# jkulhanek/tetra-nerf

Hardware: AMD Instinct MI355X
Metric: ray_tet_intersections_per_s (higher is better)
Workload: dtype f32

## Files before the change

### tetra-nerf_amd/csrc/tn_api_tracer.hip

```cpp
#include <algorithm>
#include <cmath>
#include <cstring>
#include <memory>
#include <mutex>

#include "tn_api_common.h"
#include "tn_build.h"
#include "tn_devbuf.h"
#include "tn_isosurface_core.h"
#include "tn_kernels.h"

using tn::check_loaded;
using tn::check_pow2_M;
using tn::DeviceGuard;
using tn::guarded;

struct tn_tracer {
    int device = 0;
    std::mutex mu;

    struct Mesh {
        bool loaded = false;
        tn::DeviceMesh view;
        tn::HostMesh host;
// ... 15 lines not shown
        unsigned leaf_width = 16;
        int writer_table = 0;
        bool refit_tables = false;
        int use_walk = 1;
        size_t walk_min_rays = 12288;
        bool walk_min_auto = true;
        bool dense_tails = true;
        bool literal = true;
        size_t log_cap_bytes = 0;
        int spec_fill = 0;
        unsigned spec_k0 = 0;
        tn::FillRange spec{true, 0, true, tn::FillKind::Spans, 512};
        unsigned walk_lds_kb = 26;
        tn::FillRange tail{false, 0, false, tn::FillKind::RowPerBlock, 0};
        unsigned writer_blocks = 0;
        bool hull_flat = true;
        bool small_lds = true;
        unsigned lds_cap = 0;
        unsigned verify_stride = 256;
        bool verify_risk = true;
        unsigned risk_band = 2;
        bool verify_inject = false;
        unsigned literal_sort_passes = 8;
        int cert_ends = 2;
        bool bin_rays = false;
        bool timing = false;
    } opt;

    struct Scratch {
        tn::DevBuf<uint32_t> fallback_list;
        tn::DevBuf<uint32_t> walk_n;
        tn::DevBuf<uint4> hull_entry;
        tn::DevBuf<uint2> literal_list;
        tn::DevBuf<uint4> hit_log;
        tn::DevBuf<uint32_t> verify_list;
        tn::DevBuf<uint32_t> risk_list;
        tn::DevBuf<uint32_t> ray_keys, ray_iota, ray_keys_sorted, order, walk_n_item;
        tn::DevBuf<char> sort_temp;
        static constexpr int N_CTR = 2;
        tn::DevBuf<unsigned long long> stats;
        uint32_t *fallback_count() { return reinterpret_cast<uint32_t *>(stats.p + tn::N_STATS); }
        uint32_t *literal_count() { return fallback_count() + 1; }
        uint32_t *verify_count() { return fallback_count() + 2; }
        uint32_t *risk_count() { return fallback_count() + 3; }
        static constexpr size_t stats_bytes() { return (tn::N_STATS + N_CTR) * sizeof(unsigned long long); }
        size_t last_num_rays = 0;
        bool last_walk = false;
        bool last_binned = false;
        hipStream_t last_stream = nullptr;

        template <typename T>
        static void grow(tn::DevBuf<T> &b, size_t n) { if (b.n < n) b.alloc(n); }
        void reserve(size_t R, size_t log_entries, bool verify, bool risk, size_t sort_temp_bytes = 0) {
            grow(fallback_list, R);
            if (!log_entries) return;
            grow(walk_n, R); grow(literal_list, R); grow(hull_entry, R); grow(hit_log, log_entries);
            if (verify) grow(verify_list, R);
            if (risk) grow(risk_list, R);
            if (sort_temp_bytes) {
                grow(ray_keys, R); grow(ray_iota, R); grow(ray_keys_sorted, R); grow(order, R); grow(walk_n_item, R);
                grow(sort_temp, sort_temp_bytes);
            }
        }
    } scratch;

    struct Schedule {
        hipStream_t side = nullptr;
// ... 134 lines not shown
        w.risk_band = (float)o().risk_band;
        if (binned) { w.order = s().order.p; w.walk_n_item = s().walk_n_item.p; }
        w.cert_ends = o().cert_ends == 2 ? (m.T >= tn::WALK_TET_MIN_TETS ? 1u : 3u) : (uint32_t)o().cert_ends;
        return w;
    }
    tn::WriteParams write_params(size_t base, size_t n) const {
        const tn::Rows r = rows.at(base);
        tn::WriteParams q{};
        q.num_rays = n; q.M = r.M; q.dense_tails = dense_tails ? 1u : 0u;
        q.walk_n = s().walk_n.p + base;
        q.hit_log = s().hit_log.p;
        q.cold = mesh().cold; q.tets = mesh().tets;
        q.out_cells = r.cells; q.out_bary = r.bary; q.out_dist = r.dist; q.out_verts = r.verts;
        if (binned) { q.walk_n = s().walk_n_item.p; q.order = s().order.p; }
        return q;
    }

    void fill_tails(size_t base, size_t n, uint32_t k_hi) const {
        if (!dense_tails) return;
        tn::FillRange f = o().tail;
        f.k_split = k_hi;
        tn::launch_fill(rows.at(base), n, s().walk_n.p + base, f, stream);
    }
    void pair_literal(size_t base, size_t n, hipStream_t st) const {
        if (!o().literal) return;
        tn::launch_postprocess_log(trace_params(base, n), mesh().fidt, s().hit_log.p, s().literal_list.p, s().literal_count(), n, st,
                                   binned ? s().order.p : nullptr);
    }
    void trace_listed(const uint32_t *list, const uint32_t *count, size_t max_items, hipStream_t st) const {
        tn::TraceParams q = trace_params(0, max_items);
        q.ray_list = list; q.item_count = count;
        tn::launch_trace_general(q, st);
    }

    uint32_t spec_fill_first_slot() const {
        if (!o().spec_fill || !dense_tails) return 0;
        const uint32_t M = rows.M;
        uint32_t K0 = (((uint32_t)(3.6 * std::cbrt((double)std::max<uint32_t>(mesh().T, 1u))) + 31u) & ~31u) + 32u;
        const uint32_t quarter = (3u * M / 4u) & ~31u, half = (M / 2u) & ~31u;
        if (mesh().T >= tn::WALK_TET_MIN_TETS) K0 = K0 > quarter + 32u ? 0u : quarter;
        else K0 = K0 > quarter ? 0u : (K0 + 32u > half ? half : quarter);
        if (o().spec_k0) K0 = o().spec_k0 & ~31u;
        return K0 + 32u > M ? 0u : K0;
    }

    void run_overlapped() const {
        tn_tracer::Schedule &c = t->sched;
        const bool timing = o().timing;
        const hipStream_t s_pre = timing ? stream : c.pre, s_aux = timing ? stream : c.aux, s_side = timing ? stream : c.side;
        if (timing && !c.tev[0])
// ... 33 lines not shown
        }
        mark();
        TN_HIP(hipEventRecord(c.ev_aux, s_aux));
        tn::launch_write_segments(write_params(0, R), stream, o().writer_blocks);
        mark();
        TN_HIP(hipEventRecord(c.ev_seg, stream));
        TN_HIP(hipStreamWaitEvent(s_side, c.ev_seg, 0));
        pair_literal(0, R, s_side);
        mark();
        fill_tails(0, R, K0 ? K0 : rows.M);
        mark();
        TN_HIP(hipEventRecord(c.ev_join, s_side));
        TN_HIP(hipStreamWaitEvent(stream, c.ev_join, 0));
        TN_HIP(hipStreamWaitEvent(stream, c.ev_aux, 0));
        if (o().verify_stride) trace_listed(s().verify_list.p, s().verify_count(), 64, stream);
        mark();
        c.tev_valid = timing;
    }

    void run_chunked(size_t chunk) const {
        for (size_t base = 0; base < R; base += chunk) {
            const size_t n = std::min(R - base, chunk);
            TN_HIP(hipMemsetAsync(s().literal_count(), 0, sizeof(uint32_t), stream));
            TN_HIP(hipMemsetAsync(s().risk_count(), 0, sizeof(uint32_t), stream));
            const tn::WalkParams w = walk_params(base, n);
            tn::launch_trace_walk(w, stream, 0);
            if (o().verify_stride) {
                tn::launch_verify_counts(w.t, o().verify_stride, w.walk_n, w.fallback_list, w.fallback_count, base, stream, false,
                                         o().verify_inject);
                if (verify_risk())
                    tn::launch_verify_counts(w.t, o().verify_stride, w.walk_n, w.fallback_list, w.fallback_count, base, stream, false,
                                             false, s().risk_list.p, s().risk_count(), n);
            }
            tn::launch_write_segments(write_params(base, n), stream, o().writer_blocks);
            fill_tails(base, n, rows.M);
            pair_literal(base, n, stream);
        }
        trace_listed(s().fallback_list.p, s().fallback_count(), R, stream);
    }

    void run_small_batch() const {
        uint32_t C = 64;
        const double expect = 3.6 * std::cbrt((double)std::max<uint32_t>(mesh().T, 1u));
        while (C < expect && C < rows.M) C <<= 1;
        if (o().lds_cap) C = o().lds_cap;
        tn::TraceParams p = trace_params(0, R);
        if (o().small_lds && C < rows.M) {
// ... 600 lines not shown
            o.leaf_width = (unsigned)value;
        }
        else if (k == "walk") o.use_walk = value < 0 ? 0 : (value > 2 ? 2 : value);
        else if (k == "walk_min_rays") { o.walk_min_rays = value < 0 ? 0 : (size_t)value; o.walk_min_auto = false; }
        else if (k == "dense_tails") o.dense_tails = value != 0;
        else if (k == "literal") o.literal = value != 0;
        else if (k == "spec_fill") o.spec_fill = value != 0;
        else if (k == "spec_k0") o.spec_k0 = (unsigned)value;
        else if (k == "spec_blocks") set_grid(o.spec, value);
        else if (k == "hull_flat") o.hull_flat = value != 0;
        else if (k == "writer_blocks") o.writer_blocks = (unsigned)value;
        else if (k == "fill_blocks") set_grid(o.tail, value);
        else if (k == "walk_lds_kb") o.walk_lds_kb = (unsigned)value;
        else if (k == "small_lds") o.small_lds = value != 0;
        else if (k == "lds_cap") {
            if (value < 0 || (value & (value - 1)) != 0 || (value && value < 8)) throw tn::Error("lds_cap must be 0 or a power of two >= 8");
            o.lds_cap = (unsigned)value;
        }
        else if (k == "writer_table") o.writer_table = value;
        else if (k == "refit_tables") o.refit_tables = value != 0;
        else if (k == "cert_ends") { if (value < 0 || value > 3) throw tn::Error("cert_ends must be 0 .. 3"); o.cert_ends = value; }
        else if (k == "verify_inject") o.verify_inject = value != 0;
        else if (k == "literal_sort_passes") o.literal_sort_passes = value < 0 ? 0u : (unsigned)value;
        else if (k == "verify_stride") o.verify_stride = value < 0 ? 0u : (unsigned)value;
        else if (k == "verify_risk") o.verify_risk = value != 0;
        else if (k == "risk_band") o.risk_band = value < 1 ? 1u : (unsigned)value;
        else if (k == "log_cap_mb") o.log_cap_bytes = value <= 0 ? 0 : (size_t)value << 20;
        else throw tn::Error("unknown option " + (name ? k : std::string("(null)")));
    });
}

}
```

### tetra-nerf_amd/csrc/tn_kernels.h

```cpp
#pragma once
#include "tn_common.h"
#include "tn_ray_key.h"

namespace tn {

struct Rows {
    uint32_t *num;
    uint32_t *cells;
    float *bary;
    float *dist;
    uint32_t *verts;
    uint32_t M;
    Rows at(size_t base) const {
        return Rows{num ? num + base : nullptr, cells + base * M, bary + base * M * 6, dist + base * M * 2,
                    verts ? verts + base * M * 4 : nullptr, M};
    }
};

struct TraceParams {
    const float *origins;
    const float *dirs;
    const uint32_t *faces;
    const uint32_t *face_tets;
    WideBvh bvh;
// ... 32 lines not shown
    const float4 *hull_nodes;
    const float4 *hull_tris;
    uint32_t n_hull_nodes;
    const float4 *hull_flat;
    uint32_t n_hull_groups, n_hull_leaves;
    uint32_t n_hull;
    uint4 *hull_entry;
    uint32_t *fallback_list;
    uint32_t *fallback_count;
    uint2 *literal_list;
    uint32_t *literal_count;
    uint32_t *walk_n;
    uint4 *hit_log;
    size_t ray_base;
    uint32_t *risk_list;
    uint32_t *risk_count;
    float risk_band;
    uint32_t cert_ends;
    const uint32_t *order;
    uint32_t *walk_n_item;
};
void launch_trace_walk(const WalkParams &p, hipStream_t stream, size_t lds_reserve = 0);
void launch_postprocess_log(const TraceParams &p, const WalkFid *fidt, const uint4 *hit_log, const uint2 *literal_list,
                            const uint32_t *literal_count, size_t max_items, hipStream_t stream, const uint32_t *order = nullptr);

void launch_verify_counts(const TraceParams &p, uint32_t stride, uint32_t *walk_n, uint32_t *fallback_list, uint32_t *fallback_count,
                          size_t ray_base, hipStream_t stream, bool late = false, bool inject = false, const uint32_t *ray_list = nullptr,
                          const uint32_t *list_count = nullptr, size_t max_list = 0);

struct WriteParams {
    size_t num_rays;
    uint32_t M;
    uint32_t dense_tails;
    const uint32_t *walk_n;
    const uint4 *hit_log;
    const WalkCold *cold;
    const WalkTet *tets;
    uint32_t *out_cells;
    float *out_bary;
    float *out_dist;
    uint32_t *out_verts;
    const uint32_t *order;
};
void launch_write_segments(const WriteParams &q, hipStream_t stream, unsigned max_blocks = 0);
enum class FillKind {
    Spans,
    RowPerBlock,
// ... 189 lines not shown
```

### tetra-nerf_amd/csrc/tn_trace_general.hip

```cpp
#include "tn_device.h"
#include "tn_kernels.h"

namespace tn {

namespace {

struct WaveSmem {
    uint64_t *key;
    float *hu;
    float *hv;
    uint2 *hft;
    uint32_t *stack;
    uint8_t *mark;
    uint8_t *emitf;
};

__device__ __forceinline__ WaveSmem carve(char *smem, uint32_t M) {
    WaveSmem s;
    s.key = reinterpret_cast<uint64_t *>(smem);
    s.hft = reinterpret_cast<uint2 *>(s.key + M);
    s.hu = reinterpret_cast<float *>(s.hft + (M < 32 ? 32 : M));
    s.hv = s.hu + M;
    s.stack = reinterpret_cast<uint32_t *>(s.hv + M);
    s.mark = reinterpret_cast<uint8_t *>(s.stack + STACK_CAP);
    s.emitf = s.mark + M;
    return s;
}

__device__ __forceinline__ void wave_sync() { __syncthreads(); }

__device__ void insert_overflow(WaveSmem &s, uint32_t cap, uint64_t k, float u, float v, int lane) {
    uint64_t best = 0;
    uint32_t bidx = 0;
    for (uint32_t i = lane; i < cap; i += 64) {
        const uint64_t x = s.key[i];
        if (x >= best) { best = x; bidx = i; }
    }
#pragma unroll
    for (int off = 32; off > 0; off >>= 1) {
        const uint64_t ob = __shfl_xor(best, off);
        const uint32_t oi = __shfl_xor(bidx, off);
        if (ob > best || (ob == best && oi > bidx)) { best = ob; bidx = oi; }
    }
    if (k < best && lane == 0) { s.key[bidx] = k; s.hu[bidx] = u; s.hv[bidx] = v; }
    wave_sync();
}

__device__ void postprocess_and_write(const WaveSmem &s, uint32_t nh, uint32_t M, const uint32_t *__restrict__ faces,
                                      const uint32_t *__restrict__ face_tets, uint32_t *__restrict__ out_num,
                                      uint32_t *__restrict__ out_cells, float *__restrict__ out_bary,
                                      float *__restrict__ out_dist, uint32_t *__restrict__ out_verts,
                                      unsigned long long *stats, int lane, bool compact = false) {
    for (uint32_t base = 0; base < nh; base += 512) {
        uint2 ft[8];
#pragma unroll
        for (int q = 0; q < 8; ++q) {
            const uint32_t j = base + 64 * q + lane;
            if (j < nh) ft[q] = *reinterpret_cast<const uint2 *>(face_tets + 2 * (size_t)(uint32_t)s.key[j]);
        }
#pragma unroll
        for (int q = 0; q < 8; ++q) {
            const uint32_t j = base + 64 * q + lane;
            if (j < nh) { s.hft[j] = ft[q]; s.mark[j] = 0; }
        }
    }
    wave_sync();

    bool bad = false;
    for (uint32_t j = lane; j + 1 < nh; j += 64) {
        uint32_t c;
        const float t0 = __uint_as_float((uint32_t)(s.key[j] >> 32));
        const float t1 = __uint_as_float((uint32_t)(s.key[j + 1] >> 32));
        if (!common_tet(s.hft[j], s.hft[j + 1], c)) bad = true;
        if (j + 2 < nh) {
            const float t2 = __uint_as_float((uint32_t)(s.key[j + 2] >> 32));
            if (fabsf(t1 - t0) < TN_EPS && fabsf(t2 - t1) < TN_EPS) bad = true;
        }
    }
    const bool clean = (__ballot(bad) == 0ull);

    if (clean) {
        for (uint32_t j = lane; j < nh; j += 64) {
            bool em = false;
            if (j + 1 < nh) {
                const float t0 = __uint_as_float((uint32_t)(s.key[j] >> 32));
                const float t1 = __uint_as_float((uint32_t)(s.key[j + 1] >> 32));
                em = fabsf(t0 - t1) >= TN_EPS;
            }
            s.emitf[j] = em ? 1 : 0;
        }
    } else {
        if (stats && lane == 0) atomicAdd(&stats[STAT_LITERAL_BRANCH], 1ull);
        auto Tk = [](uint64_t k) { return __uint_as_float((uint32_t)(k >> 32)); };
        auto T = [&](uint32_t j) { return Tk(s.key[j]); };
        auto ID = [&](uint32_t j) { return (uint32_t)s.key[j]; };
        uint32_t nruns = 0;
        for (uint32_t base = 0; base < nh; base += 64) {
            const uint32_t j = base + lane;
            bool start = false;
            if (j + 1 < nh) {
                const bool sj = fabsf(T(j + 1) - T(j)) < TN_EPS;
                const bool sp = j > 0 && fabsf(T(j) - T(j - 1)) < TN_EPS;
                start = sj && !sp;
            }
            const uint64_t m = __ballot(start);
            if (start) {
                const uint32_t slot = nruns + __popcll(m & lanemask_lt());
                if (slot < (uint32_t)STACK_CAP) s.stack[slot] = j;
            }
            nruns += __popcll(m);
        }
        wave_sync();
        const bool runs_fit = nruns <= (uint32_t)STACK_CAP;
        auto phase1_at = [&](uint32_t j) {
            if (ID(j) == TN_EMPTY) return;
// ... 1 lines not shown
            bool clear_self = false;
            for (uint32_t off = 1; j + off < nh && (ID(j + off) == TN_EMPTY || fabsf(T(j + off) - dn) < TN_EPS); ++off) {
                uint32_t c;
                if (ID(j + off) != TN_EMPTY && common_tet(s.hft[j], s.hft[j + off], c)) {
                    if (ID(j) != ID(j + off)) clear_self = true;
                    if (s.mark[j + off]) s.key[j + off] = (s.key[j + off] & 0xFFFFFFFF00000000ull) | TN_EMPTY;
                    else s.mark[j + off] = 1;
                }
            }
            if (clear_self && s.mark[j]) s.key[j] = (s.key[j] & 0xFFFFFFFF00000000ull) | TN_EMPTY;
            s.mark[j] = 0;
        };
        if (runs_fit) {
            for (uint32_t ci = lane; ci < nruns; ci += 64) {
                for (uint32_t j = s.stack[ci];; ++j) {
                    phase1_at(j);
                    if (!(j + 1 < nh && fabsf(T(j + 1) - T(j)) < TN_EPS)) break;
                }
            }
        } else if (lane == 0) {
            for (uint32_t j = 0; j + 1 < nh; ++j) phase1_at(j);
        }
        wave_sync();
        unsigned long long *amask = reinterpret_cast<unsigned long long *>(s.stack);
        for (uint32_t base = 0; base < nh; base += 64) {
            const uint32_t j = base + lane;
            bool anomalous = false;
            uint8_t em = 0;
            if (j + 1 < nh && ID(j) != TN_EMPTY) {
                uint32_t c;
                const bool plain = ID(j + 1) != TN_EMPTY && common_tet(s.hft[j], s.hft[j + 1], c);
                anomalous = !plain;
                em = (plain && fabsf(T(j) - T(j + 1)) >= TN_EPS) ? 1 : 0;
            }
            if (j < nh) s.emitf[j] = em;
            const uint64_t m = __ballot(anomalous);
            if (lane == 0) amask[base >> 6] = m;
        }
        wave_sync();
        if (lane == 0) {
            const uint32_t nwords = (nh + 63) >> 6;
            auto next_anomaly = [&](uint32_t from) -> uint32_t {
                for (uint32_t w = from >> 6; w < nwords; ++w) {
                    unsigned long long m = amask[w];
                    if (w == (from >> 6)) m &= ~0ull << (from & 63);
                    if (m) return (w << 6) + (uint32_t)__ffsll(m) - 1;
                }
                return nh;
            };
            uint32_t touched = 0;
            uint32_t j = next_anomaly(0);
            while (j < nh) {
                s.emitf[j] = 0;
                if (ID(j) != TN_EMPTY) {
                    uint32_t cell;
                    if (j + 1 < nh && ID(j + 1) != TN_EMPTY && common_tet(s.hft[j], s.hft[j + 1], cell)) {
                        if (fabsf(T(j) - T(j + 1)) >= TN_EPS) s.emitf[j] = 1;
                    } else {
                        const uint2 orig = s.hft[j];
                        float dn = T(j);
                        uint32_t real_off = 1;
                        for (uint32_t off = 1; j + off < nh && (real_off < 3 || ID(j + off) == TN_EMPTY || fabsf(T(j + off) - dn) < TN_EPS); ++off) {
                            if (ID(j + off) == TN_EMPTY) continue;
                            if (common_tet(orig, s.hft[j + off], cell)) {
                                if (fabsf(T(j) - T(j + off)) >= TN_EPS) s.emitf[j] = 1;
                                if (off > 1) {
                                    const uint64_t k0 = s.key[j + off]; s.key[j + off] = s.key[j + 1]; s.key[j + 1] = k0;
                                    const float u0 = s.hu[j + off]; s.hu[j + off] = s.hu[j + 1]; s.hu[j + 1] = u0;
                                    const float v0 = s.hv[j + off]; s.hv[j + off] = s.hv[j + 1]; s.hv[j + 1] = v0;
                                    const uint2 f0 = s.hft[j + off]; s.hft[j + off] = s.hft[j + 1]; s.hft[j + 1] = f0;
                                    const uint8_t m0 = s.mark[j + off]; s.mark[j + off] = s.mark[j + 1]; s.mark[j + 1] = m0;
                                    touched = j + off > touched ? j + off : touched;
                                }
                                break;
                            }
                            dn = T(j + off);
                            real_off++;
                        }
                    }
                }
                ++j;
                if (j > touched) j = next_anomaly(j);
            }
        }
    }
    wave_sync();

    uint32_t nseg = 0;
    struct FaceIds { uint32_t a[3], b[3]; bool emit; };
    auto face_ids = [&](uint32_t base) {
        FaceIds r;
        const uint32_t j = base + lane;
        r.emit = j + 1 < nh && s.emitf[j] != 0;
#pragma unroll
        for (int k = 0; k < 3; ++k) r.a[k] = r.b[k] = 0u;
        if (r.emit) {
            const uint32_t f0 = (uint32_t)s.key[j], f1 = (uint32_t)s.key[j + 1];
#pragma unroll
            for (int k = 0; k < 3; ++k) { r.a[k] = faces[3 * (size_t)f0 + k]; r.b[k] = faces[3 * (size_t)f1 + k]; }
        }
        return r;
    };
    FaceIds nxt = face_ids(0);
    for (uint32_t base = 0; base + 1 < nh; base += 64) {
        const uint32_t j = base + lane;
        const FaceIds cur = nxt;
        if (base + 65 < nh) nxt = face_ids(base + 64);
        const bool emit = cur.emit;
        const uint64_t m = __ballot(emit);
        if (emit) {
            const uint32_t slot = nseg + __popcll(m & lanemask_lt());
            const float t0 = __uint_as_float((uint32_t)(s.key[j] >> 32));
            const float t1 = __uint_as_float((uint32_t)(s.key[j + 1] >> 32));
            uint32_t cell = TN_EMPTY;
            common_tet(s.hft[j], s.hft[j + 1], cell);
            const uint32_t id1[3] = {cur.a[0], cur.a[1], cur.a[2]};
            const uint32_t id2[3] = {cur.b[0], cur.b[1], cur.b[2]};
            uint32_t vi[4];
            float b1[3], b2[3];
            combine_indices(id1, id2, s.hu[j], s.hv[j], s.hu[j + 1], s.hv[j + 1], vi, b1, b2);
            out_cells[slot] = cell;
            *reinterpret_cast<float2 *>(out_dist + 2 * (size_t)slot) = make_float2(t0, t1);
            float2 *bp = reinterpret_cast<float2 *>(out_bary + 6 * (size_t)slot);
            bp[0] = make_float2(b1[0], b1[1]);
            bp[1] = make_float2(b1[2], b2[0]);
            bp[2] = make_float2(b2[1], b2[2]);
            if (out_verts) *reinterpret_cast<uint4 *>(out_verts + 4 * (size_t)slot) = make_uint4(vi[0], vi[1], vi[2], vi[3]);
        }
        nseg += __popcll(m);
    }

    for (uint32_t j = nseg + lane; j < (compact ? nseg : M); j += 64) {
        out_cells[j] = TN_EMPTY;
        *reinterpret_cast<float2 *>(out_dist + 2 * (size_t)j) = make_float2(0.f, 0.f);
        float2 *bp = reinterpret_cast<float2 *>(out_bary + 6 * (size_t)j);
        bp[0] = make_float2(0.f, 0.f); bp[1] = make_float2(0.f, 0.f); bp[2] = make_float2(0.f, 0.f);
        if (out_verts) *reinterpret_cast<uint4 *>(out_verts + 4 * (size_t)j) = make_uint4(TN_EMPTY, TN_EMPTY, TN_EMPTY, TN_EMPTY);
    }
    if (lane == 0) *out_num = nseg;
}

__device__ void sort_hits(const WaveSmem &s, uint32_t nh, int lane) {
    uint32_t Np = 1;
    while (Np < nh) Np <<= 1;
    for (uint32_t i = nh + lane; i < Np; i += 64) s.key[i] = ~0ull;
    wave_sync();
    for (uint32_t k = 2; k <= Np; k <<= 1) {
        for (uint32_t j = k >> 1; j > 0; j >>= 1) {
            for (uint32_t tix = lane; tix < (Np >> 1); tix += 64) {
                const uint32_t i = ((tix & ~(j - 1)) << 1) | (tix & (j - 1));
                const uint32_t ij = i | j;
                const uint64_t a = s.key[i], b = s.key[ij];
                const bool up = (i & k) == 0;
                if ((a > b) == up && a != b) {
                    s.key[i] = b; s.key[ij] = a;
                    const float ua = s.hu[i], ub = s.hu[ij]; s.hu[i] = ub; s.hu[ij] = ua;
                    const float va = s.hv[i], vb = s.hv[ij]; s.hv[i] = vb; s.hv[ij] = va;
                }
            }
            wave_sync();
        }
    }
}

__device__ void sort_logged_hits(const WaveSmem &s, uint32_t nh, int lane, uint32_t max_passes) {
    for (uint32_t pass = 0; pass < max_passes; ++pass) {
        bool swapped = false;
#pragma unroll
        for (uint32_t par = 0; par < 2; ++par) {
            for (uint32_t i = 2 * (uint32_t)lane + par; i + 1 < nh; i += 128) {
                const uint64_t a = s.key[i], b = s.key[i + 1];
                if (a > b) {
                    s.key[i] = b; s.key[i + 1] = a;
                    const float ua = s.hu[i], ub = s.hu[i + 1]; s.hu[i] = ub; s.hu[i + 1] = ua;
                    const float va = s.hv[i], vb = s.hv[i + 1]; s.hv[i] = vb; s.hv[i + 1] = va;
                    swapped = true;
                }
            }
            wave_sync();
        }
        if (__ballot(swapped) == 0ull) return;
    }
    sort_hits(s, nh, lane);
}

}

__device__ uint32_t collect_hits(const WideBvh &bvh, WaveSmem &s, uint32_t M, uint32_t cap, float ox, float oy, float oz,
                                 float dx, float dy, float dz, unsigned long long *stats, int lane, bool &overflow,
                                 bool defer = false) {
    const RayPre rp = ray_pre(ox, oy, oz, dx, dy, dz);
    const float ix = safe_inv(dx), iy = safe_inv(dy), iz = safe_inv(dz);
    const float pad = 16.0f * 1.1920929e-7f * (fmaxf(fabsf(ox), fmaxf(fabsf(oy), fabsf(oz))) + bvh.scene_max);
        uint32_t nh = 0;
        overflow = false;
        bool aborted = false;

        auto test_leaf = [&](float a0, float a1, float a2, float b0, float b1, float b2, float c0, float c1, float c2,
                             uint32_t fid) {
            const SV A = shear(rp, a0, a1, a2), B = shear(rp, b0, b1, b2), C = shear(rp, c0, c1, c2);
            float t = 0.f, u = 0.f, v = 0.f;
            const bool hit = (fid != TN_EMPTY) && tri_hit_sv(A, B, C, t, u, v);
            const uint64_t m = __ballot(hit);
            const uint32_t c = __popcll(m);
            if (c) {
                const uint64_t k = ((uint64_t)__float_as_uint(t) << 32) | fid;
// ... 167 lines not shown

__global__ __launch_bounds__(64) void k_postprocess_hits(TraceParams p, const uint32_t *hit_count,
                                                         const uint32_t *hit_ids, const float *hit_t,
                                                         const float *hit_uv) {
    extern __shared__ __attribute__((aligned(16))) char smem[];
    WaveSmem s = carve(smem, p.M);
    const int lane = threadIdx.x;
    const uint32_t M = p.M;
    for (size_t ray = blockIdx.x; ray < p.num_items; ray += gridDim.x) {
        const uint32_t nh = hit_count[ray] < M ? hit_count[ray] : M;
        for (uint32_t j = lane; j < nh; j += 64) {
            s.key[j] = ((uint64_t)__float_as_uint(hit_t[ray * M + j]) << 32) | hit_ids[ray * M + j];
            s.hu[j] = hit_uv[2 * (ray * M + j)];
            s.hv[j] = hit_uv[2 * (ray * M + j) + 1];
        }
        wave_sync();
        postprocess_and_write(s, nh, M, p.faces, p.face_tets, p.out_num + ray, p.out_cells + ray * M,
                              p.out_bary + ray * M * 6, p.out_dist + ray * M * 2,
                              p.out_verts ? p.out_verts + ray * M * 4 : nullptr, p.stats, lane);
        wave_sync();
    }
}

template <bool BINNED>
__global__ __launch_bounds__(64) void k_postprocess_log(TraceParams p, const WalkFid *__restrict__ fidt,
                                                        const uint4 *__restrict__ hit_log,
                                                        const uint2 *__restrict__ literal_list,
                                                        const uint32_t *__restrict__ literal_count,
                                                        const uint32_t *__restrict__ order) {
    extern __shared__ __attribute__((aligned(16))) char smem[];
    WaveSmem s = carve(smem, p.M);
    const int lane = threadIdx.x;
    const uint32_t M = p.M;
    const size_t n_items = *literal_count;
    for (size_t it = blockIdx.x; it < n_items; it += gridDim.x) {
        const uint2 ent = literal_list[it];
        const size_t item = ent.x;
        const size_t ray = BINNED ? (size_t)order[item] : item;
        const uint32_t nh = ent.y < M ? ent.y : M - 1;
        const uint4 *lg = hit_log + (item >> 6) * (size_t)M * 64 + (item & 63);
        for (uint32_t base = 0; base < nh; base += 512) {
            uint4 e[8];
            uint32_t fid[8];
#pragma unroll
            for (int q = 0; q < 8; ++q) {
                const uint32_t j = base + 64 * q + lane;
                if (j < nh) e[q] = lg[(size_t)j * 64];
            }
#pragma unroll
            for (int q = 0; q < 8; ++q) {
                const uint32_t j = base + 64 * q + lane;
                if (j < nh) {
                    const uint32_t x = e[q].w >> 30, lo = e[q].w & 0x3FFFFFFFu;
                    fid[q] = x == 3u ? lo : fidt[lo].fid[x];
                }
            }
#pragma unroll
            for (int q = 0; q < 8; ++q) {
                const uint32_t j = base + 64 * q + lane;
                if (j < nh) {
                    s.key[j] = ((uint64_t)e[q].x << 32) | fid[q];
                    s.hu[j] = __uint_as_float(e[q].y);
                    s.hv[j] = __uint_as_float(e[q].z);
                }
            }
        }
        wave_sync();
        sort_logged_hits(s, nh, lane, p.sort_passes);
        postprocess_and_write(s, nh, M, p.faces, p.face_tets, p.out_num + ray, p.out_cells + ray * M,
                              p.out_bary + ray * M * 6, p.out_dist + ray * M * 2,
                              p.out_verts ? p.out_verts + ray * M * 4 : nullptr, p.stats, lane, p.compact_rows != 0);
        if (lane == 0 && p.stats) atomicAdd(&p.stats[STAT_REASON + REASON_LITERAL_PAIRED], 1ull);
        wave_sync();
    }
}

__global__ __launch_bounds__(64) void k_verify_counts(TraceParams p, uint32_t stride, uint32_t *__restrict__ walk_n,
                                                      uint32_t *__restrict__ fallback_list, uint32_t *__restrict__ fallback_count,
                                                      size_t ray_base, uint32_t late, uint32_t inject,
                                                      const uint32_t *__restrict__ ray_list, const uint32_t *__restrict__ list_count) {
    extern __shared__ __attribute__((aligned(16))) char smem[];
    WaveSmem s = carve(smem, p.M);
    const int lane = threadIdx.x;
    const size_t n_checks = ray_list ? (size_t)*list_count : (p.num_items + stride - 1) / stride;
    const int c_checked = ray_list ? STAT_RISK_CHECKED : STAT_REASON + REASON_VERIFY_CHECKED,
              c_bad = ray_list ? STAT_RISK_BAD : STAT_REASON + REASON_VERIFY_BAD;
    for (size_t it = blockIdx.x; it < n_checks; it += gridDim.x) {
        const size_t ray = ray_list ? (size_t)ray_list[it] : it * stride;
        if (ray_list && stride && ray % stride == 0) continue;
        const uint32_t wn_raw = walk_n[ray];
        if (wn_raw == TN_EMPTY) continue;
        const uint32_t wn = wn_raw & 0x3FFFFFFFu;
        bool overflow = false;
        const uint32_t nh = collect_hits(p.bvh, s, p.M, p.M - 1, p.origins[3 * ray], p.origins[3 * ray + 1], p.origins[3 * ray + 2],
                                         p.dirs[3 * ray], p.dirs[3 * ray + 1], p.dirs[3 * ray + 2], nullptr, lane, overflow);
        if (lane == 0) {
// ... 116 lines not shown
    const unsigned grid = (unsigned)(p.num_items < max_blocks ? p.num_items : max_blocks);
    hipLaunchKernelGGL(k_find_tetrahedra, dim3(grid), dim3(64), wave_smem(k_find_tetrahedra, p.M), stream, p, points, out_tet, out_bary, out_verts);
}

void launch_trace_general(const TraceParams &p, hipStream_t stream) {
    if (p.num_items == 0) return;
    const size_t smem = wave_smem(k_trace_general, p.lds_cap && p.lds_cap < p.M ? p.lds_cap : p.M);
    const size_t max_blocks = 256 * 16;
    const unsigned grid = (unsigned)(p.num_items < max_blocks ? p.num_items : max_blocks);
    hipLaunchKernelGGL(k_trace_general, dim3(grid), dim3(64), smem, stream, p);
}

void launch_verify_counts(const TraceParams &p, uint32_t stride, uint32_t *walk_n, uint32_t *fallback_list, uint32_t *fallback_count,
                          size_t ray_base, hipStream_t stream, bool late, bool inject, const uint32_t *ray_list,
                          const uint32_t *list_count, size_t max_list) {
    if (p.num_items == 0 || (stride == 0 && !ray_list)) return;
    const size_t smem = wave_smem(k_verify_counts, p.M);
    const size_t n_checks = ray_list ? std::min<size_t>(max_list, 256 * 16) : (p.num_items + stride - 1) / stride, max_blocks = 256 * 16;
    if (n_checks == 0) return;
    hipLaunchKernelGGL(k_verify_counts, dim3((unsigned)(n_checks < max_blocks ? n_checks : max_blocks)), dim3(64), smem, stream, p, stride,
                       walk_n, fallback_list, fallback_count, ray_base, late ? 1u : 0u, inject ? 1u : 0u, ray_list, list_count);
}

void launch_postprocess_log(const TraceParams &p, const WalkFid *fidt, const uint4 *hit_log, const uint2 *literal_list,
                            const uint32_t *literal_count, size_t max_items, hipStream_t stream, const uint32_t *order) {
    if (max_items == 0) return;
    const size_t max_blocks = 256 * 16;
    const unsigned grid = (unsigned)(max_items < max_blocks ? max_items : max_blocks);
    if (order)
        hipLaunchKernelGGL(k_postprocess_log<true>, dim3(grid), dim3(64), wave_smem(k_postprocess_log<true>, p.M), stream, p, fidt,
                           hit_log, literal_list, literal_count, order);
    else
        hipLaunchKernelGGL(k_postprocess_log<false>, dim3(grid), dim3(64), wave_smem(k_postprocess_log<false>, p.M), stream, p, fidt,
                           hit_log, literal_list, literal_count, order);
}

void launch_postprocess_hits(const TraceParams &p, const uint32_t *hit_count, const uint32_t *hit_ids,
                             const float *hit_t, const float *hit_uv, hipStream_t stream) {
    if (p.num_items == 0) return;
    const size_t smem = wave_smem(k_postprocess_hits, p.M);
    const size_t max_blocks = 256 * 16;
    const unsigned grid = (unsigned)(p.num_items < max_blocks ? p.num_items : max_blocks);
    hipLaunchKernelGGL(k_postprocess_hits, dim3(grid), dim3(64), smem, stream, p, hit_count, hit_ids, hit_t, hit_uv);
}

}
```

Baseline: 7.689 billion.

## Split literal pairing by hit count, pipeline log loads, use persistent ticketed waves

Reworks the literal-pairing postprocess kernel. Rays are split into two launches by hit count: rays with few hits run with a smaller LDS footprint so more waves fit per CU, and the remaining rays run in a second launch at full M. The kernel becomes a persistent grid sized to resident waves, pulling work through an atomic ticket counter. A PIPE variant prefetches the next ray's log entries and face ids while the current ray is sorted. It also adds compile-time-gated phase timing instrumentation and a benchmark script. The cost is an extra launch, extra counters and more complex control flow.

```diff
diff --git a/profiles/literal_pairing_bench.py b/profiles/literal_pairing_bench.py
--- /dev/null
+++ b/profiles/literal_pairing_bench.py
@@ -0,0 +1,184 @@
+#!/usr/bin/env python3
+import argparse
+import ctypes as C
+import importlib
+import json
+import os
+import statistics
+import subprocess
+import sys
+import tempfile
+import time
+from pathlib import Path
+
+import numpy as np
+
+ROOT = Path(__file__).resolve().parents[1]
+sys.path.insert(0, str(ROOT))
+KEYS = ("num_visited_cells", "visited_cells", "vertex_indices", "hit_distances", "barycentric_coordinates")
+CONFIGS = {"C6": ("1M points, 512x400 frame", 1024), "C5": ("150k points, 2^20 rays", 512), "C4": ("45k points, 800x800 frame", 512),
+           "C2": ("15k points, 800x800 frame", 512)}
+PHASES = ("log + face id reads", "sort", "face_tets", "chain test", "phase 1", "phase 2, all lanes", "phase 2, lane 0 / emit flags",
+          "emission", "tail")
+
+
+def c6_cells(n_points=1_000_000, seed=7):
+    f = Path(tempfile.gettempdir()) / f"tetranerf_literal_bench_delaunay_{n_points}_{seed}.npy"
+    if not f.exists():
+        from scipy.spatial import Delaunay
+        t0 = time.perf_counter()
+        p = np.random.default_rng(seed).random((n_points, 3)).astype(np.float32)
+        tmp = f.with_suffix(f".{os.getpid()}.npy")
+        np.save(tmp, np.ascontiguousarray(Delaunay(p.astype(np.float64)).simplices.astype(np.int32)))
+        os.replace(tmp, f)
+        print(f"# Qhull: {n_points} points in {time.perf_counter() - t0:.0f} s -> {f}", flush=True)
+    return f
+
+
+def mesh_and_rays(cfg, scenes, bench):
+    if cfg == "C6":
+        cells = np.load(c6_cells())
+        pts = np.random.default_rng(7).random((1_000_000, 3)).astype(np.float32)
+        return pts, cells, bench.frame_rays(scenes, 0, 512, 400)
+    npts, seed = {"C5": (150000, 3), "C4": (45000, 2), "C2": (15000, 0)}[cfg]
+    pts, cells = scenes.random_mesh(npts, seed)
+    return pts, cells, (scenes.outside_in_rays(1 << 20, 4) if cfg == "C5" else bench.frame_rays(scenes, 0, 800, 800))
+
+
+def checksum(out):
+    import torch
+    tot = 0
+    for k in KEYS:
+        x = out[k].reshape(-1).view(torch.int32).to(torch.int64)
+        w = (torch.arange(x.numel(), device=x.device, dtype=torch.int64) % 65521) + 1
+        tot = (tot * 31 + int((x * w).sum().item())) & 0xFFFFFFFFFFFFFFFF
+    return tot
+
+
+def child(args):
+    import torch
+    import bench
+    tn = importlib.import_module("tetra-nerf_amd")
+    scenes = importlib.import_module("tetra-nerf_amd.scenes")
+    lib = importlib.import_module("tetra-nerf_amd._lib").load()
+    dev = torch.device("cuda:0")
+    res = {}
+    for cfg in args.configs.split(","):
+        M = CONFIGS[cfg][1]
+        pts, cells, (o, d) = mesh_and_rays(cfg, scenes, bench)
+        tr = tn.TetrahedraTracer(dev)
+        tr.load_tetrahedra(torch.from_numpy(pts).to(dev), torch.from_numpy(cells).to(dev))
+        o, d = torch.from_numpy(o).to(dev), torch.from_numpy(d).to(dev)
+        out = tr.trace_rays(o, d, M)
+        torch.cuda.synchronize()
+        r = {"tets": int(len(cells)), "rays": int(o.shape[0]), "M": M, "literal_rays": tr.flag_reasons().get(13, 0),
+             "serial_rays": tr.trace_stats()["serial"], "checksum": checksum(out), "call_ms": [], "literal_ms": []}
+        del out
+        if args.phases:
+            arr = (C.c_uint64 * 16)()
+            lib.tn_debug_literal_time(arr, 1)
+            out = tr.trace_rays(o, d, M)
+            torch.cuda.synchronize()
+            lib.tn_debug_literal_time(arr, 1)
+            del out
+            r["phase_ticks"] = [int(x) for x in arr]
+        for i in range(0 if args.phases else args.allocs):
+            torch.cuda.empty_cache()
+            pad = torch.empty(((i * 37 + 5) << 20,), dtype=torch.uint8, device=dev)
+            out = tr.trace_rays(o, d, M)
+            del out
+            torch.cuda.synchronize()
+            e0, e1 = torch.cuda.Event(enable_timing=True), torch.cuda.Event(enable_timing=True)
+            e0.record()
+            for _ in range(3):
+                out = tr.trace_rays(o, d, M)
+                del out
+            e1.record()
+            torch.cuda.synchronize()
+            r["call_ms"].append(e0.elapsed_time(e1) / 3)
+            tr.set_option("timing", 1)
+            out = tr.trace_rays(o, d, M)
+            torch.cuda.synchronize()
+            r["literal_ms"].append(tr.trace_timings()["literal_pairing"])
+            tr.set_option("timing", 0)
+            del out, pad
+        res[cfg] = r
+        del tr, o, d
+        torch.cuda.empty_cache()
+    print("RESULT " + json.dumps(res), flush=True)
+
+
+def run_child(lib, args, extra=()):
+    env = dict(os.environ)
+    if lib:
+        env["TETRANERF_HIP_LIB"] = str(Path(lib).resolve())
+    cmd = [sys.executable, str(Path(__file__).resolve()), "--child", "--configs", args.configs, "--allocs", str(args.allocs), *extra]
+    p = subprocess.run(cmd, env=env, stdout=subprocess.PIPE, stderr=subprocess.PIPE, text=True, timeout=args.child_timeout)
+    line = [l for l in p.stdout.splitlines() if l.startswith("RESULT ")]
+    if p.returncode != 0 or not line:
+        sys.stderr.write(p.stderr[-4000:])
+        raise SystemExit(f"child process of {lib or 'the tree library'} failed with status {p.returncode}")
+    return json.loads(line[-1][7:])
+
+
+def main():
+    ap = argparse.ArgumentParser()
+    ap.add_argument("--parent-lib")
+    ap.add_argument("--new-lib", action="append", default=None)
+    ap.add_argument("--rounds", type=int, default=2)
+    ap.add_argument("--allocs", type=int, default=5)
+    ap.add_argument("--configs", default="C6,C5,C4,C2")
+    ap.add_argument("--phases", action="store_true")
+    ap.add_argument("--child", action="store_true")
+    ap.add_argument("--child-timeout", type=float, default=900.0)
+    args = ap.parse_args()
+    if args.child:
+        return child(args)
+    if "C6" in args.configs.split(","):
+        c6_cells()
+    if args.phases:
+        res = run_child(args.new_lib[0] if args.new_lib else None, args, ("--phases",))
+        for cfg, r in res.items():
+            t = r["phase_ticks"]
+            rays = max(t[0], 1)
+            print(f"{cfg} ({CONFIGS[cfg][0]}, {r['tets']} tets, M = {r['M']}): {t[0]} literal rays of {r['rays']}, {t[10] / rays:.0f} hits per ray, "
+                  f"{t[12]} took the literal branch, {t[11] / rays:.2f} anomalous steps on lane 0 per ray")
+            tot = sum(t[1:10])
+            for k, name in enumerate(PHASES, 1):
+                print(f"    {name:32s} {t[k] / rays / 100:9.2f} us per ray  {100 * t[k] / max(tot, 1):5.1f} %")
+            print(f"    {'sum':32s} {tot / rays / 100:9.2f} us per ray (100 MHz wall clock, lane 0, summed over resident waves)")
+        return
+    if not args.parent_lib:
+        raise SystemExit("--parent-lib is required (or --phases)")
+    libs = {"parent": args.parent_lib}
+    for i, spec in enumerate(args.new_lib or [None]):
+        name, _, path = spec.rpartition("=") if spec else ("", "", None)
+        libs[name or ("new" if i == 0 else f"new{i}")] = path
+    runs = {name: [] for name in libs}
+    for rnd in range(args.rounds):
+        for which in (list(libs) if rnd % 2 == 0 else list(libs)[::-1]):
+            runs[which].append(run_child(libs[which], args))
+            print(f"# round {rnd} {which} done", flush=True)
+    med = statistics.median
+    for cfg in args.configs.split(","):
+        a = [r[cfg] for r in runs["parent"]]
+        same = len({r[cfg]["checksum"] for rs in runs.values() for r in rs}) == 1
+        print(f"{cfg} ({CONFIGS[cfg][0]}, {a[0]['tets']} tets, {a[0]['rays']} rays, M = {a[0]['M']}; {a[0]['literal_rays']} literal rays, "
+              f"{a[0]['serial_rays']} on the serial branch): outputs of all builds {'bit-identical (checksum)' if same else 'DIFFER'}")
+        for key, name in (("call_ms", "whole call"), ("literal_ms", "literal_pairing (timing)")):
+            pa = [x for r in a for x in r[key]]
+            span = max(med(r[key]) for r in a) - min(med(r[key]) for r in a)
+            print(f"    {name:26s} parent {med(pa):7.3f} ms ({min(pa):.3f} .. {max(pa):.3f}; per-process medians span {span:.3f})")
+            prev = med(pa)
+            for which in list(libs)[1:]:
+                pb = [x for r in runs[which] for x in r[cfg][key]]
+                gain = med(pa) - med(pb)
+                verdict = ("beyond" if abs(gain) > max(span, max(pa) - min(pa)) else
+                           "beyond the per-process span of" if abs(gain) > span else "within")
+                print(f"    {'':26s} {which:8s} {med(pb):7.3f} ms ({min(pb):.3f} .. {max(pb):.3f})   {-100 * gain / med(pa):+6.1f} % of the parent, "
+                      f"{med(pb) - prev:+.3f} ms on the arm before   {verdict} the parent's spread")
+                prev = med(pb)
+
+
+if __name__ == "__main__":
+    main()
diff --git a/tetra-nerf_amd/csrc/tn_api_tracer.hip b/tetra-nerf_amd/csrc/tn_api_tracer.hip
--- a/tetra-nerf_amd/csrc/tn_api_tracer.hip
+++ b/tetra-nerf_amd/csrc/tn_api_tracer.hip
@@ -61,6 +61,7 @@
         unsigned risk_band = 2;
         bool verify_inject = false;
         unsigned literal_sort_passes = 8;
+        unsigned literal_lds_cap = 0;
         int cert_ends = 2;
         bool bin_rays = false;
         bool timing = false;
@@ -76,12 +77,13 @@
         tn::DevBuf<uint32_t> risk_list;
         tn::DevBuf<uint32_t> ray_keys, ray_iota, ray_keys_sorted, order, walk_n_item;
         tn::DevBuf<char> sort_temp;
-        static constexpr int N_CTR = 2;
+        static constexpr int N_CTR = 3;
         tn::DevBuf<unsigned long long> stats;
         uint32_t *fallback_count() { return reinterpret_cast<uint32_t *>(stats.p + tn::N_STATS); }
         uint32_t *literal_count() { return fallback_count() + 1; }
         uint32_t *verify_count() { return fallback_count() + 2; }
         uint32_t *risk_count() { return fallback_count() + 3; }
+        uint32_t *literal_tickets() { return fallback_count() + 4; }
         static constexpr size_t stats_bytes() { return (tn::N_STATS + N_CTR) * sizeof(unsigned long long); }
         size_t last_num_rays = 0;
         bool last_walk = false;
@@ -262,10 +264,16 @@
         f.k_split = k_hi;
         tn::launch_fill(rows.at(base), n, s().walk_n.p + base, f, stream);
     }
+    uint32_t literal_lds_cap() const {
+        if (o().literal_lds_cap) return std::min<uint32_t>(o().literal_lds_cap, rows.M);
+        const uint32_t C = (((uint32_t)std::ceil(3.6 * std::cbrt((double)std::max<uint32_t>(mesh().T, 1u))) + 63u) & ~63u) + 64u;
+        if (C >= rows.M || tn::postprocess_log_waves_per_cu(C) < tn::postprocess_log_waves_per_cu(rows.M) + 2) return rows.M;
+        return C;
+    }
     void pair_literal(size_t base, size_t n, hipStream_t st) const {
         if (!o().literal) return;
         tn::launch_postprocess_log(trace_params(base, n), mesh().fidt, s().hit_log.p, s().literal_list.p, s().literal_count(), n, st,
-                                   binned ? s().order.p : nullptr);
+                                   binned ? s().order.p : nullptr, literal_lds_cap(), s().literal_tickets());
     }
     void trace_listed(const uint32_t *list, const uint32_t *count, size_t max_items, hipStream_t st) const {
         tn::TraceParams q = trace_params(0, max_items);
@@ -345,7 +353,7 @@
         for (size_t base = 0; base < R; base += chunk) {
             const size_t n = std::min(R - base, chunk);
             TN_HIP(hipMemsetAsync(s().literal_count(), 0, sizeof(uint32_t), stream));
-            TN_HIP(hipMemsetAsync(s().risk_count(), 0, sizeof(uint32_t), stream));
+            TN_HIP(hipMemsetAsync(s().risk_count(), 0, 3 * sizeof(uint32_t), stream));
             const tn::WalkParams w = walk_params(base, n);
             tn::launch_trace_walk(w, stream, 0);
             if (o().verify_stride) {
@@ -992,6 +1000,10 @@
         else if (k == "cert_ends") { if (value < 0 || value > 3) throw tn::Error("cert_ends must be 0 .. 3"); o.cert_ends = value; }
         else if (k == "verify_inject") o.verify_inject = value != 0;
         else if (k == "literal_sort_passes") o.literal_sort_passes = value < 0 ? 0u : (unsigned)value;
+        else if (k == "literal_lds_cap") {
+            if (value < 0) throw tn::Error("literal_lds_cap must be 0 (from the mesh size) or a number of hit slots");
+            o.literal_lds_cap = (unsigned)value;
+        }
         else if (k == "verify_stride") o.verify_stride = value < 0 ? 0u : (unsigned)value;
         else if (k == "verify_risk") o.verify_risk = value != 0;
         else if (k == "risk_band") o.risk_band = value < 1 ? 1u : (unsigned)value;
diff --git a/tetra-nerf_amd/csrc/tn_kernels.h b/tetra-nerf_amd/csrc/tn_kernels.h
--- a/tetra-nerf_amd/csrc/tn_kernels.h
+++ b/tetra-nerf_amd/csrc/tn_kernels.h
@@ -78,7 +78,9 @@
 };
 void launch_trace_walk(const WalkParams &p, hipStream_t stream, size_t lds_reserve = 0);
 void launch_postprocess_log(const TraceParams &p, const WalkFid *fidt, const uint4 *hit_log, const uint2 *literal_list,
-                            const uint32_t *literal_count, size_t max_items, hipStream_t stream, const uint32_t *order = nullptr);
+                            const uint32_t *literal_count, size_t max_items, hipStream_t stream, const uint32_t *order,
+                            uint32_t lds_cap, uint32_t *tickets);
+unsigned postprocess_log_waves_per_cu(uint32_t cap);
 
 void launch_verify_counts(const TraceParams &p, uint32_t stride, uint32_t *walk_n, uint32_t *fallback_list, uint32_t *fallback_count,
                           size_t ray_base, hipStream_t stream, bool late = false, bool inject = false, const uint32_t *ray_list = nullptr,
diff --git a/tetra-nerf_amd/csrc/tn_trace_general.hip b/tetra-nerf_amd/csrc/tn_trace_general.hip
--- a/tetra-nerf_amd/csrc/tn_trace_general.hip
+++ b/tetra-nerf_amd/csrc/tn_trace_general.hip
@@ -29,6 +29,19 @@
 
 __device__ __forceinline__ void wave_sync() { __syncthreads(); }
 
+#ifndef TN_LITERAL_DIAG
+#define TN_LITERAL_DIAG 0
+#endif
+struct LitClock { unsigned long long prev; };
+#if TN_LITERAL_DIAG
+__device__ unsigned long long g_lit_time[16];
+#define LIT_LAP(clk, k) do { if ((clk) && lane == 0) { const unsigned long long t_ = wall_clock64(); atomicAdd(&g_lit_time[k], t_ - (clk)->prev); (clk)->prev = t_; } } while (0)
+#define LIT_COUNT(clk, k, n) do { if ((clk) && lane == 0) atomicAdd(&g_lit_time[k], (unsigned long long)(n)); } while (0)
+#else
+#define LIT_LAP(clk, k) ((void)0)
+#define LIT_COUNT(clk, k, n) ((void)0)
+#endif
+
 __device__ void insert_overflow(WaveSmem &s, uint32_t cap, uint64_t k, float u, float v, int lane) {
     uint64_t best = 0;
     uint32_t bidx = 0;
@@ -50,7 +63,7 @@
                                       const uint32_t *__restrict__ face_tets, uint32_t *__restrict__ out_num,
                                       uint32_t *__restrict__ out_cells, float *__restrict__ out_bary,
                                       float *__restrict__ out_dist, uint32_t *__restrict__ out_verts,
-                                      unsigned long long *stats, int lane, bool compact = false) {
+                                      unsigned long long *stats, int lane, bool compact = false, LitClock *clk = nullptr) {
     for (uint32_t base = 0; base < nh; base += 512) {
         uint2 ft[8];
 #pragma unroll
@@ -65,6 +78,7 @@
         }
     }
     wave_sync();
+    LIT_LAP(clk, 3);
 
     bool bad = false;
     for (uint32_t j = lane; j + 1 < nh; j += 64) {
@@ -78,6 +92,7 @@
         }
     }
     const bool clean = (__ballot(bad) == 0ull);
+    LIT_LAP(clk, 4);
 
     if (clean) {
         for (uint32_t j = lane; j < nh; j += 64) {
@@ -91,6 +106,7 @@
         }
     } else {
         if (stats && lane == 0) atomicAdd(&stats[STAT_LITERAL_BRANCH], 1ull);
+        LIT_COUNT(clk, 12, 1);
         auto Tk = [](uint64_t k) { return __uint_as_float((uint32_t)(k >> 32)); };
         auto T = [&](uint32_t j) { return Tk(s.key[j]); };
         auto ID = [&](uint32_t j) { return (uint32_t)s.key[j]; };
@@ -138,6 +154,7 @@
             for (uint32_t j = 0; j + 1 < nh; ++j) phase1_at(j);
         }
         wave_sync();
+        LIT_LAP(clk, 5);
         unsigned long long *amask = reinterpret_cast<unsigned long long *>(s.stack);
         for (uint32_t base = 0; base < nh; base += 64) {
             const uint32_t j = base + lane;
@@ -154,6 +171,7 @@
             if (lane == 0) amask[base >> 6] = m;
         }
         wave_sync();
+        LIT_LAP(clk, 6);
         if (lane == 0) {
             const uint32_t nwords = (nh + 63) >> 6;
             auto next_anomaly = [&](uint32_t from) -> uint32_t {
@@ -167,6 +185,7 @@
             uint32_t touched = 0;
             uint32_t j = next_anomaly(0);
             while (j < nh) {
+                LIT_COUNT(clk, 11, 1);
                 s.emitf[j] = 0;
                 if (ID(j) != TN_EMPTY) {
                     uint32_t cell;
@@ -201,6 +220,7 @@
         }
     }
     wave_sync();
+    LIT_LAP(clk, 7);
 
     uint32_t nseg = 0;
     struct FaceIds { uint32_t a[3], b[3]; bool emit; };
@@ -245,6 +265,7 @@
         }
         nseg += __popcll(m);
     }
+    LIT_LAP(clk, 8);
 
     for (uint32_t j = nseg + lane; j < (compact ? nseg : M); j += 64) {
         out_cells[j] = TN_EMPTY;
@@ -254,6 +275,7 @@
         if (out_verts) *reinterpret_cast<uint4 *>(out_verts + 4 * (size_t)j) = make_uint4(TN_EMPTY, TN_EMPTY, TN_EMPTY, TN_EMPTY);
     }
     if (lane == 0) *out_num = nseg;
+    LIT_LAP(clk, 9);
 }
 
 __device__ void sort_hits(const WaveSmem &s, uint32_t nh, int lane) {
@@ -279,6 +301,35 @@
     }
 }
 
+__device__ void sort_hits_in_place(const WaveSmem &s, uint32_t nh, int lane) {
+    uint32_t Np = 1;
+    while (Np < nh) Np <<= 1;
+    auto exchange = [&](uint32_t i, uint32_t ij) {
+        if (ij >= nh) return;
+        const uint64_t a = s.key[i], b = s.key[ij];
+        if (a > b) {
+            s.key[i] = b; s.key[ij] = a;
+            const float ua = s.hu[i], ub = s.hu[ij]; s.hu[i] = ub; s.hu[ij] = ua;
+            const float va = s.hv[i], vb = s.hv[ij]; s.hv[i] = vb; s.hv[ij] = va;
+        }
+    };
+    for (uint32_t k = 2; k <= Np; k <<= 1) {
+        const uint32_t h = k >> 1;
+        for (uint32_t tix = lane; tix < (Np >> 1); tix += 64) {
+            const uint32_t i = ((tix & ~(h - 1)) << 1) | (tix & (h - 1));
+            exchange(i, i ^ (k - 1));
+        }
+        wave_sync();
+        for (uint32_t j = k >> 2; j > 0; j >>= 1) {
+            for (uint32_t tix = lane; tix < (Np >> 1); tix += 64) {
+                const uint32_t i = ((tix & ~(j - 1)) << 1) | (tix & (j - 1));
+                exchange(i, i | j);
+            }
+            wave_sync();
+        }
+    }
+}
+
 __device__ void sort_logged_hits(const WaveSmem &s, uint32_t nh, int lane, uint32_t max_passes) {
     for (uint32_t pass = 0; pass < max_passes; ++pass) {
         bool swapped = false;
@@ -297,7 +348,7 @@
         }
         if (__ballot(swapped) == 0ull) return;
     }
-    sort_hits(s, nh, lane);
+    sort_hits_in_place(s, nh, lane);
 }
 
 }
@@ -511,56 +562,136 @@
     }
 }
 
-template <bool BINNED>
-__global__ __launch_bounds__(64) void k_postprocess_log(TraceParams p, const WalkFid *__restrict__ fidt,
+#if TN_LITERAL_DIAG
+extern "C" int tn_debug_literal_time(unsigned long long out[16], int reset) {
+    if (hipMemcpyFromSymbol(out, HIP_SYMBOL(g_lit_time), sizeof(unsigned long long) * 16) != hipSuccess) return 1;
+    if (reset) { unsigned long long z[16] = {}; if (hipMemcpyToSymbol(HIP_SYMBOL(g_lit_time), z, sizeof z) != hipSuccess) return 1; }
+    return 0;
+}
+#endif
+
+template <bool BINNED, bool PIPE>
+__global__ __launch_bounds__(64, PIPE ? 2 : 3) void k_postprocess_log(TraceParams p, const WalkFid *__restrict__ fidt,
                                                         const uint4 *__restrict__ hit_log,
                                                         const uint2 *__restrict__ literal_list,
                                                         const uint32_t *__restrict__ literal_count,
-                                                        const uint32_t *__restrict__ order) {
+                                                        const uint32_t *__restrict__ order, uint32_t cap, uint32_t min_hits,
+                                                        uint32_t *__restrict__ ticket) {
     extern __shared__ __attribute__((aligned(16))) char smem[];
-    WaveSmem s = carve(smem, p.M);
+    WaveSmem s = carve(smem, cap);
     const int lane = threadIdx.x;
     const uint32_t M = p.M;
-    const size_t n_items = *literal_count;
-    for (size_t it = blockIdx.x; it < n_items; it += gridDim.x) {
-        const uint2 ent = literal_list[it];
-        const size_t item = ent.x;
-        const size_t ray = BINNED ? (size_t)order[item] : item;
-        const uint32_t nh = ent.y < M ? ent.y : M - 1;
-        const uint4 *lg = hit_log + (item >> 6) * (size_t)M * 64 + (item & 63);
-        for (uint32_t base = 0; base < nh; base += 512) {
-            uint4 e[8];
-            uint32_t fid[8];
+    const uint32_t n_items = *literal_count;
+    uint4 e[8];
+    uint32_t fid[8];
+    size_t r_item = 0, r_ray = 0;
+    uint32_t r_nh = 0;
+    bool r_mine = false;
+    auto request_log = [&](uint2 ent) {
+        r_item = ent.x;
+        r_nh = ent.y < M ? ent.y : M - 1;
+        r_mine = r_nh < cap && r_nh >= min_hits;
+        if (!r_mine) return;
+        r_ray = BINNED ? (size_t)order[r_item] : r_item;
+        if constexpr (PIPE) {
+            const uint4 *lg = hit_log + (r_item >> 6) * (size_t)M * 64 + (r_item & 63);
 #pragma unroll
             for (int q = 0; q < 8; ++q) {
-                const uint32_t j = base + 64 * q + lane;
-                if (j < nh) e[q] = lg[(size_t)j * 64];
-            }
-#pragma unroll
-            for (int q = 0; q < 8; ++q) {
-                const uint32_t j = base + 64 * q + lane;
-                if (j < nh) {
-                    const uint32_t x = e[q].w >> 30, lo = e[q].w & 0x3FFFFFFFu;
-                    fid[q] = x == 3u ? lo : fidt[lo].fid[x];
-                }
-            }
-#pragma unroll
-            for (int q = 0; q < 8; ++q) {
-                const uint32_t j = base + 64 * q + lane;
-                if (j < nh) {
-                    s.key[j] = ((uint64_t)e[q].x << 32) | fid[q];
-                    s.hu[j] = __uint_as_float(e[q].y);
-                    s.hv[j] = __uint_as_float(e[q].z);
-                }
-            }
-        }
-        wave_sync();
-        sort_logged_hits(s, nh, lane, p.sort_passes);
-        postprocess_and_write(s, nh, M, p.faces, p.face_tets, p.out_num + ray, p.out_cells + ray * M,
-                              p.out_bary + ray * M * 6, p.out_dist + ray * M * 2,
-                              p.out_verts ? p.out_verts + ray * M * 4 : nullptr, p.stats, lane, p.compact_rows != 0);
-        if (lane == 0 && p.stats) atomicAdd(&p.stats[STAT_REASON + REASON_LITERAL_PAIRED], 1ull);
-        wave_sync();
+                const uint32_t j = 64 * q + lane;
+                if (j < r_nh) e[q] = lg[(size_t)j * 64];
+            }
+        }
+    };
+    auto request_fid = [&]() {
+        if (!r_mine) return;
+#pragma unroll
+        for (int q = 0; q < 8; ++q) {
+            const uint32_t j = 64 * q + lane;
+            if (j < r_nh) {
+                const uint32_t x = e[q].w >> 30, lo = e[q].w & 0x3FFFFFFFu;
+                fid[q] = x == 3u ? lo : fidt[lo].fid[x];
+            }
+        }
+    };
+    auto draw = [&]() { return lane == 0 ? 2u * gridDim.x + atomicAdd(ticket, 1u) : 0u; };
+    const uint2 none = make_uint2(0u, 0u);
+    uint32_t cur = blockIdx.x, nxt = blockIdx.x + gridDim.x;
+    uint2 ent_cur = cur < n_items ? literal_list[cur] : none, ent_nxt = nxt < n_items ? literal_list[nxt] : none;
+    if (PIPE && cur < n_items) {
+        request_log(ent_cur);
+        request_fid();
+    }
+    while (cur < n_items) {
+        if constexpr (!PIPE) request_log(ent_cur);
+        const size_t item = r_item, ray = r_ray;
+        const uint32_t nh = r_nh;
+        const bool mine = r_mine, has_next = nxt < n_items;
+        const uint32_t drawn = has_next ? draw() : 0u;
+#if TN_LITERAL_DIAG
+        LitClock clock{(unsigned long long)wall_clock64()}, *clk = mine ? &clock : nullptr;
+#else
+        LitClock *clk = nullptr;
+#endif
+        if (mine) {
+            LIT_COUNT(clk, 0, 1); LIT_COUNT(clk, 10, nh);
+            if constexpr (PIPE) {
+#pragma unroll
+                for (int q = 0; q < 8; ++q) {
+                    const uint32_t j = 64 * q + lane;
+                    if (j < nh) {
+                        s.key[j] = ((uint64_t)e[q].x << 32) | fid[q];
+                        s.hu[j] = __uint_as_float(e[q].y);
+                        s.hv[j] = __uint_as_float(e[q].z);
+                    }
+                }
+            }
+            const uint4 *lg = hit_log + (item >> 6) * (size_t)M * 64 + (item & 63);
+            for (uint32_t base = PIPE ? 512 : 0; base < nh; base += 512) {
+                uint4 e2[8];
+                uint32_t fid2[8];
+#pragma unroll
+                for (int q = 0; q < 8; ++q) {
+                    const uint32_t j = base + 64 * q + lane;
+                    if (j < nh) e2[q] = lg[(size_t)j * 64];
+                }
+#pragma unroll
+                for (int q = 0; q < 8; ++q) {
+                    const uint32_t j = base + 64 * q + lane;
+                    if (j < nh) {
+                        const uint32_t x = e2[q].w >> 30, lo = e2[q].w & 0x3FFFFFFFu;
+                        fid2[q] = x == 3u ? lo : fidt[lo].fid[x];
+                    }
+                }
+#pragma unroll
+                for (int q = 0; q < 8; ++q) {
+                    const uint32_t j = base + 64 * q + lane;
+                    if (j < nh) {
+                        s.key[j] = ((uint64_t)e2[q].x << 32) | fid2[q];
+                        s.hu[j] = __uint_as_float(e2[q].y);
+                        s.hv[j] = __uint_as_float(e2[q].z);
+                    }
+                }
+            }
+            wave_sync();
+            LIT_LAP(clk, 1);
+        }
+        if (PIPE && has_next) request_log(ent_nxt);
+        if (mine) {
+            sort_logged_hits(s, nh, lane, p.sort_passes);
+            LIT_LAP(clk, 2);
+        }
+        const uint32_t nxt2 = has_next ? __shfl(drawn, 0) : n_items;
+        const uint2 ent_nxt2 = nxt2 < n_items ? literal_list[nxt2] : none;
+        if (PIPE && has_next) request_fid();
+        if (mine) {
+            postprocess_and_write(s, nh, M, p.faces, p.face_tets, p.out_num + ray, p.out_cells + ray * M,
+                                  p.out_bary + ray * M * 6, p.out_dist + ray * M * 2,
+                                  p.out_verts ? p.out_verts + ray * M * 4 : nullptr, p.stats, lane, p.compact_rows != 0, clk);
+            if (lane == 0 && p.stats) atomicAdd(&p.stats[STAT_REASON + REASON_LITERAL_PAIRED], 1ull);
+            wave_sync();
+        }
+        cur = nxt; nxt = nxt2;
+        ent_cur = ent_nxt; ent_nxt = ent_nxt2;
     }
 }
 
@@ -723,17 +854,31 @@
                        walk_n, fallback_list, fallback_count, ray_base, late ? 1u : 0u, inject ? 1u : 0u, ray_list, list_count);
 }
 
+static size_t postprocess_log_by_lds(uint32_t cap) { return (160 * 1024) / trace_general_smem_bytes(cap); }
+unsigned postprocess_log_waves_per_cu(uint32_t cap) {
+    const size_t by_lds = postprocess_log_by_lds(cap);
+    return (unsigned)std::min<size_t>(by_lds <= 8 ? 8 : 12, by_lds);
+}
+
 void launch_postprocess_log(const TraceParams &p, const WalkFid *fidt, const uint4 *hit_log, const uint2 *literal_list,
-                            const uint32_t *literal_count, size_t max_items, hipStream_t stream, const uint32_t *order) {
+                            const uint32_t *literal_count, size_t max_items, hipStream_t stream, const uint32_t *order,
+                            uint32_t lds_cap, uint32_t *tickets) {
     if (max_items == 0) return;
-    const size_t max_blocks = 256 * 16;
-    const unsigned grid = (unsigned)(max_items < max_blocks ? max_items : max_blocks);
-    if (order)
-        hipLaunchKernelGGL(k_postprocess_log<true>, dim3(grid), dim3(64), wave_smem(k_postprocess_log<true>, p.M), stream, p, fidt,
-                           hit_log, literal_list, literal_count, order);
-    else
-        hipLaunchKernelGGL(k_postprocess_log<false>, dim3(grid), dim3(64), wave_smem(k_postprocess_log<false>, p.M), stream, p, fidt,
-                           hit_log, literal_list, literal_count, order);
+    int device = 0, cus = 0;
+    TN_HIP(hipGetDevice(&device));
+    TN_HIP(hipDeviceGetAttribute(&cus, hipDeviceAttributeMultiprocessorCount, device));
+    auto launch = [&](uint32_t cap, uint32_t min_hits, uint32_t *ticket) {
+        const bool pipe = postprocess_log_by_lds(cap) <= 8;
+        const auto kernel = order ? (pipe ? k_postprocess_log<true, true> : k_postprocess_log<true, false>)
+                                  : (pipe ? k_postprocess_log<false, true> : k_postprocess_log<false, false>);
+        const size_t smem = wave_smem(kernel, cap);
+        const size_t resident = (size_t)postprocess_log_waves_per_cu(cap) * (size_t)std::max(cus, 1);
+        hipLaunchKernelGGL(kernel, dim3((unsigned)std::min(max_items, resident)), dim3(64), smem, stream, p, fidt, hit_log, literal_list,
+                           literal_count, order, cap, min_hits, ticket);
+    };
+    const uint32_t C = lds_cap && lds_cap < p.M ? lds_cap : p.M;
+    launch(C, 0u, tickets);
+    if (C < p.M) launch(p.M, C, tickets + 1);
 }
 
 void launch_postprocess_hits(const TraceParams &p, const uint32_t *hit_count, const uint32_t *hit_ids,
```

Measured after the change: 7.760 billion (median of 2 runs). About the same (+0.9%).
